# simonfuhrmann/mve

Hardware: NVIDIA H100
Metric: mvs_depth_pixels_per_second (higher is better)
Workload: dtype f32

## Files before the change

### mve_b200/csrc/patch_opt.cuh

```cuda
#pragma once
#if defined(B200MVS_HOST_EMU)
#include "simt_emu.h"
#else
#include <cuda_runtime.h>
#endif
#include <stdint.h>
#include <cstddef>

namespace b200mvs {

constexpr int MAX_LEVELS = 12;
constexpr int MAX_GLOBAL = 32;
constexpr int MAX_LOCAL = 4;
constexpr unsigned FULL = 0xffffffffu;
constexpr int NS = 25;
constexpr int CENTER = 12;
constexpr int LUT_REP = 32;
constexpr int LUT_STRIDE = 64;

struct alignas(16) LevelParams {
    float ax, ay, cx, cy;
    int w, h;
    int pitch;
    int pad;
    const uchar4* img;
    const uint4* quad;
};
static_assert(sizeof(LevelParams) == 48, "LevelParams layout");

struct alignas(16) ViewParams {
    float campos[3];
    float inv_ax0;
    float w2c[12];
    float rot[9];
    int nlevels;
    int valid;
    int pad;
    LevelParams lv[MAX_LEVELS];
};
static_assert(offsetof(ViewParams, lv) % 16 == 0, "ViewParams layout");

struct DevSettings {
    float min_ncc, min_parallax, accept_ncc, min_refine_diff;
    unsigned max_iterations, nr_recon_neighbors;
    int scale, use_color_scale;
};

struct JobParams {
    int ref_view, W, H, n_global;
    int gview[MAX_GLOBAL];
    float ki0, ki2, ki4, ki5;
    const uchar4* ref_img;
    int ref_pitch;
    int tiles_x;
    float* depth; float* conf; float* dz; float* normal;
    unsigned* slots;
    unsigned long long* sel;
    long long tile_base;
};

struct PatchIn  { int x, y; float depth, dzI, dzJ; unsigned slots; };
struct PatchOut { float conf, depth, dzI, dzJ, nx, ny, nz; unsigned slots; int iterations; int flags; };

#if defined(B200MVS_HOST_EMU)
__device__ __forceinline__ float rcp_fast(float x) { return 1.f / x; }
__device__ __forceinline__ float rsqrt_fast(float x) { return 1.f / sqrtf(x); }
#else
__device__ __forceinline__ float rcp_fast(float x) { float r; asm("rcp.approx.ftz.f32 %0, %1;" : "=f"(r) : "f"(x)); return r; }
__device__ __forceinline__ float rsqrt_fast(float x) { float r; asm("rsqrt.approx.ftz.f32 %0, %1;" : "=f"(r) : "f"(x)); return r; }
#endif

template <int K> __device__ __forceinline__ float lut_k(const float* table, unsigned lane4, unsigned w)
{
    static_assert(LUT_REP == 32 && LUT_STRIDE == 64, "offset arithmetic assumes 32 lanes and 256-byte rows");
#if defined(B200MVS_HOST_EMU)
    const unsigned off = (((w >> (8 * K)) & 0xFFu) << 8) | lane4;
#else
    const unsigned off = __byte_perm(w, lane4, 0x6504u | ((unsigned)K << 4));
#endif
    return *reinterpret_cast<const float*>(reinterpret_cast<const char*>(table) + off);
}

__device__ __forceinline__ float plx_weight(float p)
{
    if (p < 0.f || p > 180.f) return 0.f;
    const float sigma = (p <= 20.f) ? 5.f : 15.f;
    const float dlt = p - 20.f;
    return expf(-(dlt * dlt) / (2.f * sigma * sigma));
}
__device__ __forceinline__ float clamp1(float v) { return v < -1.f ? -1.f : (v > 1.f ? 1.f : v); }
__device__ __forceinline__ float deg_acos(float dp) { return acosf(dp) * 180.f / 3.141592653589793f; }

}
```

### mve_b200/csrc/patch_thread.cuh

```cuda
#pragma once
#include "patch_opt.cuh"

namespace b200mvs {

#if defined(B200MVS_SWEEP_MIX) && !defined(B200MVS_HOST_EMU)
__device__ unsigned long long g_sweep_mix[128];
__device__ __forceinline__ void count_sweep_mix(unsigned kind)
{
    const unsigned act = __activemask();
    const unsigned same = __match_any_sync(act, kind);
    const int lane = (int)(threadIdx.x & 31u);
    const unsigned firsts = __ballot_sync(act, (__ffs(same) - 1) == lane);
    atomicAdd(&g_sweep_mix[64 + (kind & 63u)], 1ull);
    if (lane == __ffs(act) - 1) {
        atomicAdd(&g_sweep_mix[__popc(firsts) & 31], 1ull);
        atomicAdd(&g_sweep_mix[32], 1ull);
        atomicAdd(&g_sweep_mix[33], (unsigned long long)__popc(act));
    }
}
#endif

struct PatchT {
    const DevSettings* st;
    const ViewParams* views;
#if defined(B200MVS_HOST_EMU)
    const float* lut_tab;
    unsigned lane4;
#endif
    const JobParams* job;
    unsigned xy;
    float u0x, u0y, u0z;
    float uax, uay, uaz;
    float ubx, uby, ubz;
    float c0x, c0y, c0z;
    float mx0, mx1, mx2;
    float crx, cry, crz;
    float cpx, cpy, cpz;
    float mfp, inv_mfp;
    float mm, inv_mm, sqrDevX;
    float depth, dzI, dzJ;
    unsigned avail;
    int iter;
    unsigned n_sets;
    unsigned pk;
    unsigned selp;
    float cs[MAX_LOCAL][3];
    float ncc[MAX_LOCAL];


    struct PassOut { float num, den, nX0, nX1, nX2; };
    enum Stage { LVS_CTOR, CTOR, FIRST, PRE, POST, LVS_REPL, REPL, DONE };
    enum : unsigned {
        F_REF_OK = 1u << 0,
        F_OPTI = 1u << 1, F_CONVERGED = 1u << 2, F_LVS_OK = 1u << 3, F_VIEW_REMOVED = 1u << 4, F_WAS_NORMAL = 1u << 5,
        F_NORMAL = 1u << 6, F_SINGULAR = 1u << 7, F_HAS_NORMAL = 1u << 8, F_HAS_NCC = 1u << 9
    };
    static constexpr int SH_STAGE = 10, SH_NSEL = 13, SH_COL = 16, SH_DER = 20, SH_DF = 24;
    __device__ __forceinline__ bool is(unsigned f) const { return (pk & f) != 0u; }
    __device__ __forceinline__ void put(unsigned f, bool v) { pk = v ? (pk | f) : (pk & ~f); }
    __device__ __forceinline__ int stage() const { return (int)((pk >> SH_STAGE) & 7u); }
    __device__ __forceinline__ void set_stage(int v) { pk = (pk & ~(7u << SH_STAGE)) | ((unsigned)v << SH_STAGE); }
    __device__ __forceinline__ int nsel() const { return (int)((pk >> SH_NSEL) & 7u); }
    __device__ __forceinline__ void set_nsel(int v) { pk = (pk & ~(7u << SH_NSEL)) | ((unsigned)v << SH_NSEL); }
    __device__ __forceinline__ int sel(int k) const { return (int)((selp >> (8 * k)) & 0xFFu); }
    __device__ __forceinline__ int px() const { return (int)(xy & 0xFFFFu); }
    __device__ __forceinline__ int py() const { return (int)(xy >> 16); }

    template <typename T> static __device__ __forceinline__ T get4(const T (&a)[MAX_LOCAL], int k)
    {
        return k == 0 ? a[0] : (k == 1 ? a[1] : (k == 2 ? a[2] : a[3]));
    }
    template <typename T> static __device__ __forceinline__ void set4(T (&a)[MAX_LOCAL], int k, T v)
    {
#pragma unroll
        for (int i = 0; i < MAX_LOCAL; ++i) if (i == k) a[i] = v;
    }

    __device__ __forceinline__ unsigned lane_offset() const
    {
#if defined(B200MVS_HOST_EMU)
        return lane4;
#else
        return (threadIdx.x & 31u) << 2;
#endif
    }
    __device__ __forceinline__ const float* table() const
    {
#if defined(B200MVS_HOST_EMU)
        return lut_tab;
#else
        extern __shared__ float b200mvs_dyn_smem[];
        return b200mvs_dyn_smem;
#endif
    }

    __device__ __forceinline__ void sample_ray(float di, float dj, float& ux, float& uy, float& uz, float& inv) const
    {
        ux = u0x + di * uax + dj * ubx;
        uy = u0y + di * uay + dj * uby;
        uz = u0z + di * uaz + dj * ubz;
        inv = rsqrt_fast(ux * ux + uy * uy + uz * uz);
    }

    __device__ __forceinline__ void compute_points()
    {
        bool bad = false;
#pragma unroll 5
        for (int k = 0; k < NS; ++k) {
            const float t = depth + (float)(k % 5 - 2) * dzI + (float)(k / 5 - 2) * dzJ;
            bad |= t <= 0.f;
        }
        if (bad) pk &= ~F_REF_OK;
        cpx = c0x + depth * crx;
        cpy = c0y + depth * cry;
        cpz = c0z + depth * crz;
        const ViewParams* rv = &views[job->ref_view];
        const float z = __ldg(&rv->w2c[8]) * cpx + __ldg(&rv->w2c[9]) * cpy + __ldg(&rv->w2c[10]) * cpz + __ldg(&rv->w2c[11]);
        mfp = z * job->ki0;
        inv_mfp = rcp_fast(mfp);
    }

    __device__ __forceinline__ void init_sampler(int x, int y)
    {
        const float* const lut_tab = table();
        const unsigned lane4 = lane_offset();
        pk &= ~F_REF_OK; mm = 0.f; inv_mm = 0.f; sqrDevX = 0.f;
        mx0 = mx1 = mx2 = 0.f;
        crx = cry = crz = cpx = cpy = cpz = mfp = inv_mfp = 0.f;
        if (x - 2 < 0 || y - 2 < 0 || x + 2 > job->W - 1 || y + 2 > job->H - 1) return;
        {
            const ViewParams* rv = &views[job->ref_view];
            const float r0 = __ldg(&rv->rot[0]), r1 = __ldg(&rv->rot[1]), r2 = __ldg(&rv->rot[2]), r3 = __ldg(&rv->rot[3]), r4 = __ldg(&rv->rot[4]);
            const float r5 = __ldg(&rv->rot[5]), r6 = __ldg(&rv->rot[6]), r7 = __ldg(&rv->rot[7]), r8 = __ldg(&rv->rot[8]);
            const float vx = job->ki0 * ((float)x + 0.5f) + job->ki2, vy = job->ki4 * ((float)y + 0.5f) + job->ki5;
            u0x = r0 * vx + r3 * vy + r6; u0y = r1 * vx + r4 * vy + r7; u0z = r2 * vx + r5 * vy + r8;
            uax = r0 * job->ki0; uay = r1 * job->ki0; uaz = r2 * job->ki0;
            ubx = r3 * job->ki4; uby = r4 * job->ki4; ubz = r5 * job->ki4;
            c0x = __ldg(&rv->campos[0]); c0y = __ldg(&rv->campos[1]); c0z = __ldg(&rv->campos[2]);
            const float inv = rsqrt_fast(u0x * u0x + u0y * u0y + u0z * u0z);
            crx = u0x * inv; cry = u0y * inv; crz = u0z * inv;
        }
        pk |= F_REF_OK;
        const uchar4* row = job->ref_img + (size_t)(y - 2) * job->ref_pitch + (x - 2);
        float s0 = 0.f, s1 = 0.f, s2 = 0.f;
#pragma unroll 1
        for (int j = 0; j < 5; ++j) {
#pragma unroll
            for (int i = 0; i < 5; ++i) {
                const unsigned t = reinterpret_cast<const unsigned*>(row)[i];
                s0 += lut_k<0>(lut_tab, lane4, t); s1 += lut_k<1>(lut_tab, lane4, t); s2 += lut_k<2>(lut_tab, lane4, t);
            }
            row += job->ref_pitch;
        }
        mm = (s0 + s1 + s2) / (3.f * NS);
        if (mm < 0.01f || mm > 0.99f) { pk &= ~F_REF_OK; return; }
        inv_mm = 1.f / mm;
        mx0 = (s0 * inv_mm) / (float)NS; mx1 = (s1 * inv_mm) / (float)NS; mx2 = (s2 * inv_mm) / (float)NS;
        row = job->ref_img + (size_t)(y - 2) * job->ref_pitch + (x - 2);
        float dev = 0.f;
#pragma unroll 1
        for (int j = 0; j < 5; ++j) {
#pragma unroll
            for (int i = 0; i < 5; ++i) {
                const unsigned t = reinterpret_cast<const unsigned*>(row)[i];
                const float e0 = lut_k<0>(lut_tab, lane4, t) * inv_mm - mx0, e1 = lut_k<1>(lut_tab, lane4, t) * inv_mm - mx1, e2 = lut_k<2>(lut_tab, lane4, t) * inv_mm - mx2;
                dev += e0 * e0 + e1 * e1 + e2 * e2;
            }
            row += job->ref_pitch;
        }
        sqrDevX = dev;
        compute_points();
    }

    __device__ __forceinline__ void update()
    {
        pk |= F_REF_OK;
        compute_points();
    }

    __device__ __forceinline__ void pass(bool candidates, bool cs_pending, bool want_ncc, bool want_normal, float* cand, PassOut& po)
    {
        const float* const lut_tab = table();
        const unsigned lane4 = lane_offset();
        const float u0x = this->u0x, u0y = this->u0y, u0z = this->u0z, uax = this->uax, uay = this->uay, uaz = this->uaz;
        const float ubx = this->ubx, uby = this->uby, ubz = this->ubz;
        const float depth = this->depth, dzI = this->dzI, dzJ = this->dzJ;
        const float inv_mm = this->inv_mm;
        const JobParams* const job = this->job;
        float num = 0.f, den = 0.f;
        double D0 = 0.0, D1 = 0.0, D2 = 0.0, D3 = 0.0, D4 = 0.0, D5 = 0.0, E0 = 0.0, E1 = 0.0, E2 = 0.0;
        bool cs_active = cs_pending && st->use_color_scale;
        if (!candidates) pk &= want_ncc ? ~((0xFFu << SH_COL) | (0xFu << SH_DF)) : ~(0xFFu << SH_COL);
        const int count = candidates ? job->n_global : nsel();
        const int x0 = px(), y0 = py();
        const float pv0 = mx0 * mm, pv1 = mx1 * mm, pv2 = mx2 * mm;
#pragma unroll 1
        for (int k = 0; k < count; ++k) {
            int slot = k;
            if (candidates) { if (!((avail >> k) & 1u)) continue; }
            else slot = sel(k);
            const ViewParams* V = &views[job->gview[slot]];
            ++n_sets;
            float c0 = 1.f, c1 = 1.f, c2 = 1.f;
            if (!candidates) {
                c0 = k == 0 ? cs[0][0] : (k == 1 ? cs[1][0] : (k == 2 ? cs[2][0] : cs[3][0]));
                c1 = k == 0 ? cs[0][1] : (k == 1 ? cs[1][1] : (k == 2 ? cs[2][1] : cs[3][1]));
                c2 = k == 0 ? cs[0][2] : (k == 1 ? cs[1][2] : (k == 2 ? cs[2][2] : cs[3][2]));
            }
            unsigned r = 0u;
            float A0x = 0.f, A0y = 0.f, A0z = 0.f, W0x = 0.f, W0y = 0.f, W0z = 0.f, Wax = 0.f, Way = 0.f, Waz = 0.f, Wbx = 0.f, Wby = 0.f, Wbz = 0.f;
            float Lax = 0.f, Lay = 0.f, Lcx = 0.f, Lcy = 0.f, wm1 = 0.f, hm1 = 0.f, dd = 0.f, step = 0.f;
            int Lpitch = 0;
            const uint4* Lquad = nullptr;
            bool dok = false;
            {
                const float4 wa = __ldg(reinterpret_cast<const float4*>(&V->w2c[0]));
                const float4 wb = __ldg(reinterpret_cast<const float4*>(&V->w2c[4]));
                const float4 wc = __ldg(reinterpret_cast<const float4*>(&V->w2c[8]));
                A0x = wa.x * c0x + wa.y * c0y + wa.z * c0z + wa.w;
                A0y = wb.x * c0x + wb.y * c0y + wb.z * c0z + wb.w;
                A0z = wc.x * c0x + wc.y * c0y + wc.z * c0z + wc.w;
                W0x = wa.x * u0x + wa.y * u0y + wa.z * u0z; W0y = wb.x * u0x + wb.y * u0y + wb.z * u0z; W0z = wc.x * u0x + wc.y * u0y + wc.z * u0z;
                Wax = wa.x * uax + wa.y * uay + wa.z * uaz; Way = wb.x * uax + wb.y * uay + wb.z * uaz; Waz = wc.x * uax + wc.y * uay + wc.z * uaz;
                Wbx = wa.x * ubx + wa.y * uby + wa.z * ubz; Wby = wb.x * ubx + wb.y * uby + wb.z * ubz; Wbz = wc.x * ubx + wc.y * uby + wc.z * ubz;
                const float nz = wc.x * cpx + wc.y * cpy + wc.z * cpz + wc.w;
                const float nfp = nz * __ldg(&V->inv_ax0);
                if (mfp > 0.f && !(nfp <= 0.f)) {
                    float ratio = nfp * inv_mfp;
                    int l = 0;
                    while (ratio < 0.5f) { ++l; ratio *= 2.f; }
                    const int nl = __ldg(&V->nlevels);
                    if (l > nl - 1) l = nl - 1;
                    const float4 kk = __ldg(reinterpret_cast<const float4*>(&V->lv[l].ax));
                    const int4 g = __ldg(reinterpret_cast<const int4*>(&V->lv[l].w));
                    Lax = kk.x; Lay = kk.y; Lcx = kk.z; Lcy = kk.w; wm1 = (float)(g.x - 1); hm1 = (float)(g.y - 1); Lpitch = g.z;
                    Lquad = reinterpret_cast<const uint4*>(__ldg(reinterpret_cast<const unsigned long long*>(&V->lv[l].quad)));
                    const float inv0 = rsqrt_fast(u0x * u0x + u0y * u0y + u0z * u0z);
                    const float sa = depth * inv0, sb = (depth + 1.f) * inv0;
                    const float hz1 = A0z + sa * W0z, hz2 = A0z + sb * W0z;
                    const float i1 = rcp_fast(hz1), i2 = rcp_fast(hz2);
                    const float ddx = (Lax * (A0x + sb * W0x) + Lcx * hz2) * i2 - (Lax * (A0x + sa * W0x) + Lcx * hz1) * i1;
                    const float ddy = (Lay * (A0y + sb * W0y) + Lcy * hz2) * i2 - (Lay * (A0y + sa * W0y) + Lcy * hz1) * i1;
                    const float dd2 = ddx * ddx + ddy * ddy;
                    dd = dd2 * rsqrt_fast(dd2);
                    dok = dd > 0.f;
                    step = rcp_fast(dd);
                    r = dok ? 3u : 1u;
                    if (!dok) dd = 0.f;
                }
            }
            const bool need_ncc = candidates || want_ncc;
            const bool cs_view = !candidates && cs_active;
            float nccv = -1.f;
#pragma unroll 1
            for (int rep = 0; rep < 2 && r != 0u; ++rep) {
                const bool second = rep == 1;
                if (second && !(cs_view && want_normal && (r & 2u))) break;
                const bool gn = !candidates && (r & 2u) && (second || !(cs_view && want_normal));
                const bool nrm = gn && want_normal;
#if defined(B200MVS_SWEEP_MIX) && !defined(B200MVS_HOST_EMU)
                {
                    const bool g_ = !candidates && (r & 2u);
                    count_sweep_mix((!second && need_ncc ? 1u : 0u) | (!second && cs_view ? 2u : 0u) |
                                    (g_ && !second && cs_view && !want_normal ? 4u : 0u) | (g_ && (second || !cs_view) ? 8u : 0u) |
                                    (g_ && (second || !cs_view) && want_normal ? 16u : 0u) | (candidates ? 32u : 0u));
                }
#endif
                float Sya = 0.f, Syb = 0.f, Syc = 0.f, Syya = 0.f, Syyb = 0.f, Syyc = 0.f, Smya = 0.f, Smyb = 0.f, Smyc = 0.f;
                float Sdma = 0.f, Sdmb = 0.f, Sdmc = 0.f, Sdna = 0.f, Sdnb = 0.f, Sdnc = 0.f, Sdda = 0.f, Sddb = 0.f, Sddc = 0.f;
                float A1 = 0.f, A2 = 0.f, A3 = 0.f, A4 = 0.f, A5 = 0.f, B1 = 0.f, B2 = 0.f;
                bool oob = false;
                const uchar4* mptr = job->ref_img + (size_t)(y0 - 2) * job->ref_pitch + (x0 - 2);
                const int mskip = job->ref_pitch - 5;
                float ndi = -2.f, ndj = -2.f;
                float nfx = 0.f, nfy = 0.f, ngx = 0.f, ngy = 0.f;
                uint4 nQ = make_uint4(0u, 0u, 0u, 0u);
                unsigned nmt = 0u;
                bool nvalid = false;
#define B200MVS_STAGE_NEXT() do { \
                    const float ux_ = u0x + ndi * uax + ndj * ubx, uy_ = u0y + ndi * uay + ndj * uby, uz_ = u0z + ndi * uaz + ndj * ubz; \
                    const float inv_ = rsqrt_fast(ux_ * ux_ + uy_ * uy_ + uz_ * uz_); \
                    const float t_ = depth + ndi * dzI + ndj * dzJ; \
                    const float s1_ = t_ * inv_; \
                    const float wx_ = W0x + ndi * Wax + ndj * Wbx, wy_ = W0y + ndi * Way + ndj * Wby, wz_ = W0z + ndi * Waz + ndj * Wbz; \
                    const float hx_ = A0x + s1_ * wx_, hy_ = A0y + s1_ * wy_, hz_ = A0z + s1_ * wz_; \
                    const float ih_ = rcp_fast(hz_); \
                    const float qx_ = (Lax * hx_ + Lcx * hz_) * ih_ - 0.5f; \
                    const float qy_ = (Lay * hy_ + Lcy * hz_) * ih_ - 0.5f; \
                    nvalid = qx_ > 0.f && qx_ < wm1 && qy_ > 0.f && qy_ < hm1; \
                    if (nvalid) { \
                        ngx = 0.f; ngy = 0.f; \
                        if (dok) { \
                            const float s2_ = s1_ + step * inv_; \
                            const float kx_ = A0x + s2_ * wx_, ky_ = A0y + s2_ * wy_, kz_ = A0z + s2_ * wz_; \
                            const float ik_ = rcp_fast(kz_); \
                            ngx = (Lax * kx_ + Lcx * kz_) * ik_ - 0.5f - qx_; \
                            ngy = (Lay * ky_ + Lcy * kz_) * ik_ - 0.5f - qy_; \
                        } \
                        const int left_ = (int)floorf(qx_), top_ = (int)floorf(qy_); \
                        nfx = qx_ - (float)left_; nfy = qy_ - (float)top_; \
                        noff = (unsigned)top_ * (unsigned)Lpitch + (unsigned)left_; \
                        nQ = __ldg(Lquad + noff); \
                        nmt = *reinterpret_cast<const unsigned*>(mptr); \
                    } \
                } while (0)
                unsigned noff = 0u;
                B200MVS_STAGE_NEXT();
#ifdef B200MVS_T1_UNROLL2
#pragma unroll 2
#else
#pragma unroll 1
#endif
                for (int k = 0; k < NS; ++k) {
                    if (!nvalid) { oob = true; break; }
                    const float di = ndi, dj = ndj, fx = nfx, fy = nfy, gx = ngx, gy = ngy;
                    const uint4 Q = nQ;
                    const unsigned mt = nmt;
                    if (k + 1 < NS) {
                        ndi += 1.f; ++mptr;
                        if (ndi > 2.f) { ndi = -2.f; ndj += 1.f; mptr += mskip; }
                        B200MVS_STAGE_NEXT();
                    }
                    {
                        const float m[3] = {lut_k<0>(lut_tab, lane4, mt) * inv_mm, lut_k<1>(lut_tab, lane4, mt) * inv_mm, lut_k<2>(lut_tab, lane4, mt) * inv_mm};
                        float a[3], b[3], c[3], e[3];
                        a[0] = lut_k<0>(lut_tab, lane4, Q.x); a[1] = lut_k<1>(lut_tab, lane4, Q.x); a[2] = lut_k<2>(lut_tab, lane4, Q.x);
                        b[0] = lut_k<0>(lut_tab, lane4, Q.y); b[1] = lut_k<1>(lut_tab, lane4, Q.y); b[2] = lut_k<2>(lut_tab, lane4, Q.y);
                        c[0] = lut_k<0>(lut_tab, lane4, Q.z); c[1] = lut_k<1>(lut_tab, lane4, Q.z); c[2] = lut_k<2>(lut_tab, lane4, Q.z);
                        e[0] = lut_k<0>(lut_tab, lane4, Q.w); e[1] = lut_k<1>(lut_tab, lane4, Q.w); e[2] = lut_k<2>(lut_tab, lane4, Q.w);
                        float n[3], d[3];
#pragma unroll
                        for (int ch = 0; ch < 3; ++ch) {
                            const float x0_ = (1.f - fx) * a[ch] + fx * b[ch];
                            const float x3_ = (1.f - fx) * c[ch] + fx * e[ch];
                            n[ch] = (1.f - fy) * x0_ + fy * x3_;
                            const float der = gx * (b[ch] - a[ch]) + gy * (c[ch] - a[ch]) + (gy * fx + gx * fy) * (a[ch] - b[ch] - c[ch] + e[ch]);
                            d[ch] = der * dd;
                        }
                        const float y0_ = n[0] - pv0, y1_ = n[1] - pv1, y2_ = n[2] - pv2;
                        Sya += y0_; Syb += y1_; Syc += y2_;
                        Syya += y0_ * y0_; Syyb += y1_ * y1_; Syyc += y2_ * y2_;
                        Smya += m[0] * y0_; Smyb += m[1] * y1_; Smyc += m[2] * y2_;
                        Sdma += d[0] * m[0]; Sdmb += d[1] * m[1]; Sdmc += d[2] * m[2];
                        Sdna += d[0] * n[0]; Sdnb += d[1] * n[1]; Sdnc += d[2] * n[2];
                        Sdda += d[0] * d[0]; Sddb += d[1] * d[1]; Sddc += d[2] * d[2];
                        if (nrm) {
                            const float g0 = c0 * d[0], g1 = c1 * d[1], g2 = c2 * d[2];
                            const float q = g0 * g0 + g1 * g1 + g2 * g2;
                            const float s = g0 * (m[0] - c0 * n[0]) + g1 * (m[1] - c1 * n[1]) + g2 * (m[2] - c2 * n[2]);
                            const float qi = di * q, qj = dj * q;
                            A1 += qi; A2 += qj; A3 += di * qi; A4 += dj * qi; A5 += dj * qj;
                            B1 += di * s; B2 += dj * s;
                        }
                    }
                }
#undef B200MVS_STAGE_NEXT
                if (oob) { r = 0u; break; }
                if (!second && need_ncc) {
                    const float inv_n = 1.f / (float)NS;
                    const float sqrDevY = (Syya - Sya * Sya * inv_n) + (Syyb - Syb * Syb * inv_n) + (Syyc - Syc * Syc * inv_n);
                    const float Sen = (Smya - mx0 * Sya) + (Smyb - mx1 * Syb) + (Smyc - mx2 * Syc);
                    const float p = sqrDevX * sqrDevY;
                    nccv = p > 0.f ? Sen * rsqrt_fast(p) : -1.f;
                }
                if (!second && cs_view) {
                    const float Mna = Smya + pv0 * ((float)NS * mx0), Mnb = Smyb + pv1 * ((float)NS * mx1), Mnc = Smyc + pv2 * ((float)NS * mx2);
                    const float Nna = Syya + pv0 * (2.f * Sya + (float)NS * pv0), Nnb = Syyb + pv1 * (2.f * Syb + (float)NS * pv1);
                    const float Nnc = Syyc + pv2 * (2.f * Syc + (float)NS * pv2);
                    float cc[3] = {c0, c1, c2};
                    const float ab[3] = {Mna - c0 * Nna, Mnb - c1 * Nnb, Mnc - c2 * Nnc};
                    const float aa[3] = {Nna, Nnb, Nnc};
#pragma unroll
                    for (int ch = 0; ch < 3; ++ch) {
                        if ((double)fabsf(aa[ch]) > 1e-6) {
                            cc[ch] += ab[ch] * rcp_fast(aa[ch]);
                            if ((double)cc[ch] > 1e3) pk &= ~F_OPTI;
                        } else
                            pk &= ~F_OPTI;
                    }
                    c0 = cc[0]; c1 = cc[1]; c2 = cc[2];
#pragma unroll
                    for (int i = 0; i < MAX_LOCAL; ++i) if (i == k) { cs[i][0] = c0; cs[i][1] = c1; cs[i][2] = c2; }
                }
                if (gn) {
                    const float vn = c0 * (Sdma - c0 * Sdna) + c1 * (Sdmb - c1 * Sdnb) + c2 * (Sdmc - c2 * Sdnc);
                    const float vd = c0 * c0 * Sdda + c1 * c1 * Sddb + c2 * c2 * Sddc;
                    num += vn; den += vd;
                    if (nrm) {
                        D0 += (double)vd; D1 += (double)A1; D2 += (double)A2; D3 += (double)A3; D4 += (double)A4; D5 += (double)A5;
                        E0 += (double)vn; E1 += (double)B1; E2 += (double)B2;
                    }
                }
            }
            if (!candidates) {
                if (r & 1u) pk |= 1u << (SH_COL + k);
                if (r & 2u) pk |= 1u << (SH_DER + k);
                if (cs_active && !(r & 1u)) cs_active = false;
                if (want_ncc) {
                    const float v = (r & 1u) ? nccv : -1.f;
                    if (fabsf(v - get4(ncc, k)) > st->min_refine_diff) pk |= 1u << (SH_DF + k);
                    set4(ncc, k, v);
                }
            } else {
                const float v = (r & 1u) ? nccv : -1.f;
                if (v < st->min_ncc) avail &= ~(1u << k);
                else cand[k] = v;
            }
        }
        if (candidates) return;
        po.num = num; po.den = den;
        put(F_HAS_NORMAL, want_normal);
        put(F_HAS_NCC, want_ncc);
        if (want_normal) {
            const double m[9] = {D0, D1, D2, D1, D3, D4, D2, D4, D5};
            const double det = m[0] * m[4] * m[8] + m[1] * m[5] * m[6] + m[2] * m[3] * m[7]
                             - m[2] * m[4] * m[6] - m[1] * m[3] * m[8] - m[0] * m[5] * m[7];
            put(F_SINGULAR, det == 0.0);
            double inv[9];
            inv[0] = m[4] * m[8] - m[5] * m[7];
            inv[1] = m[2] * m[7] - m[1] * m[8];
            inv[2] = m[1] * m[5] - m[2] * m[4];
            inv[3] = m[5] * m[6] - m[3] * m[8];
            inv[4] = m[0] * m[8] - m[2] * m[6];
            inv[5] = m[2] * m[3] - m[0] * m[5];
            inv[6] = m[3] * m[7] - m[4] * m[6];
            inv[7] = m[1] * m[6] - m[0] * m[7];
            inv[8] = m[0] * m[4] - m[1] * m[3];
#pragma unroll
            for (int q = 0; q < 9; ++q) inv[q] /= det;
            po.nX0 = (float)(inv[0] * E0 + inv[1] * E1 + inv[2] * E2);
            po.nX1 = (float)(inv[3] * E0 + inv[4] * E1 + inv[5] * E2);
            po.nX2 = (float)(inv[6] * E0 + inv[7] * E1 + inv[8] * E2);
        }
    }

    __device__ __forceinline__ bool all_der_ok() const { return ((pk >> SH_DER) & 0xFu) == ((1u << nsel()) - 1u); }

    __device__ __forceinline__ bool depth_step(const PassOut& po)
    {
        if (!all_der_ok()) { pk &= ~F_OPTI; return false; }
        if (po.den > 0.f) {
            depth += po.num / po.den;
            update();
            put(F_OPTI, is(F_REF_OK));
            return true;
        }
        return false;
    }

    __device__ __forceinline__ bool normal_step(const PassOut& po)
    {
        if (!all_der_ok()) { pk &= ~F_OPTI; return false; }
        if (is(F_SINGULAR)) { pk &= ~F_OPTI; return false; }
        dzI += po.nX1; dzJ += po.nX2; depth += po.nX0;
        update();
        put(F_OPTI, is(F_REF_OK));
        return true;
    }

    __device__ __forceinline__ void sel_erase_mask(unsigned mask)
    {
        const int n = nsel();
        int cnt = 0;
        unsigned packed = 0xFFFFFFFFu;
#pragma unroll
        for (int k = 0; k < MAX_LOCAL; ++k) {
            if (k < n && !((mask >> k) & 1u)) {
                const unsigned s8 = (selp >> (8 * k)) & 0xFFu;
                const float a = cs[k][0], b = cs[k][1], c = cs[k][2], v = ncc[k];
                packed = (packed & ~(0xFFu << (8 * cnt))) | (s8 << (8 * cnt));
#pragma unroll
                for (int q = 0; q < MAX_LOCAL; ++q) if (q == cnt) { cs[q][0] = a; cs[q][1] = b; cs[q][2] = c; ncc[q] = v; }
                ++cnt;
            }
        }
        selp = packed;
        set_nsel(cnt);
    }
    __device__ __forceinline__ void sel_insert(int slot, float cs_init)
    {
        const int n = nsel();
        int pos = 0;
#pragma unroll
        for (int k = 0; k < MAX_LOCAL; ++k) if (k < n && sel(k) < slot) ++pos;
#pragma unroll
        for (int q = MAX_LOCAL - 1; q > 0; --q)
            if (q > pos && q <= n) { cs[q][0] = cs[q - 1][0]; cs[q][1] = cs[q - 1][1]; cs[q][2] = cs[q - 1][2]; ncc[q] = ncc[q - 1]; }
#pragma unroll
        for (int q = 0; q < MAX_LOCAL; ++q) if (q == pos) { cs[q][0] = cs[q][1] = cs[q][2] = cs_init; ncc[q] = 0.f; }
        const unsigned low = pos == 0 ? 0u : (selp & (0xFFFFFFFFu >> (32 - 8 * pos)));
        const unsigned high = pos >= 3 ? 0u : ((selp >> (8 * pos)) << (8 * (pos + 1)));
        selp = low | ((unsigned)slot << (8 * pos)) | high;
        set_nsel(n + 1);
    }

    __device__ __forceinline__ void cand_geometry(int slot, float rdx, float rdy, float rdz,
                                                  float& vdx, float& vdy, float& vdz, float& epx, float& epy, float& epz, float& nfp) const
    {
        const ViewParams* V = &views[job->gview[slot]];
        vdx = cpx - __ldg(&V->campos[0]); vdy = cpy - __ldg(&V->campos[1]); vdz = cpz - __ldg(&V->campos[2]);
        const float nn = sqrtf(vdx * vdx + vdy * vdy + vdz * vdz);
        vdx /= nn; vdy /= nn; vdz /= nn;
        epx = vdy * rdz - vdz * rdy; epy = vdz * rdx - vdx * rdz; epz = vdx * rdy - vdy * rdx;
        const float en = sqrtf(epx * epx + epy * epy + epz * epz);
        epx /= en; epy /= en; epz /= en;
        const float z = __ldg(&V->w2c[8]) * cpx + __ldg(&V->w2c[9]) * cpy + __ldg(&V->w2c[10]) * cpz + __ldg(&V->w2c[11]);
        nfp = z * __ldg(&V->inv_ax0);
    }

    __device__ __forceinline__ void lvs_greedy(const float* cand)
    {
        const unsigned N = st->nr_recon_neighbors;
        const float cs_init = 1.f / mm;
        float rdx = cpx - c0x, rdy = cpy - c0y, rdz = cpz - c0z;
        {
            const float nn = sqrtf(rdx * rdx + rdy * rdy + rdz * rdz);
            rdx /= nn; rdy /= nn; rdz /= nn;
        }
        const int G = job->n_global;
        bool found = true;
        while ((unsigned)nsel() < N && found) {
            found = false;
            float maxScore = 0.f;
            int maxView = 0;
#pragma unroll 1
            for (int c = 0; c < G; ++c) {
                if (!((avail >> c) & 1u)) continue;
                float vdx, vdy, vdz, epx, epy, epz, nfp;
                cand_geometry(c, rdx, rdy, rdz, vdx, vdy, vdz, epx, epy, epz, nfp);
                float score = cand[c];
                if (mfp / nfp < 0.5f) score *= 0.01f;
                float dp = clamp1(rdx * vdx + rdy * vdy + rdz * vdz);
                score *= plx_weight(deg_acos(dp));
                const int ns = nsel();
#pragma unroll 1
                for (int k = 0; k < ns; ++k) {
                    float sx, sy, sz, ex, ey, ez, sfp;
                    cand_geometry(sel(k), rdx, rdy, rdz, sx, sy, sz, ex, ey, ez, sfp);
                    dp = clamp1(sx * vdx + sy * vdy + sz * vdz);
                    score *= plx_weight(deg_acos(dp));
                    dp = clamp1(epx * ex + epy * ey + epz * ez);
                    float angle = fabsf(deg_acos(dp));
                    if (angle > 90.f) angle = 180.f - angle;
                    angle = fmaxf(angle, 1.f);
                    if (angle < st->min_parallax) score *= angle / st->min_parallax;
                }
                if (score > maxScore) { maxScore = score; maxView = c; found = true; }
            }
            if (found) {
                sel_insert(maxView, cs_init);
                avail &= ~(1u << maxView);
            }
        }
        if ((unsigned)nsel() == N) pk |= F_LVS_OK;
    }

    __device__ __forceinline__ void begin(const JobParams* j, const PatchIn& in)
    {
        job = j;
        xy = ((unsigned)in.x & 0xFFFFu) | ((unsigned)in.y << 16);
        depth = in.depth; dzI = in.dzI; dzJ = in.dzJ;
        iter = 0;
        pk = F_OPTI | F_SINGULAR | ((unsigned)DONE << SH_STAGE);
        avail = 0u;
        u0x = u0y = u0z = uax = uay = uaz = ubx = uby = ubz = c0x = c0y = c0z = 0.f;
        init_sampler(in.x, in.y);
        selp = in.slots;
        int n = 0;
#pragma unroll
        for (int k = 0; k < MAX_LOCAL; ++k) {
            if (sel(k) != 0xFF) n = k + 1;
            cs[k][0] = cs[k][1] = cs[k][2] = 0.f; ncc[k] = 0.f;
        }
        set_nsel(n);
        if (!is(F_REF_OK)) { pk &= ~F_OPTI; return; }
        const unsigned N = st->nr_recon_neighbors;
        if ((unsigned)n == N) pk |= F_LVS_OK;
        else if ((unsigned)n > N) {
            n = 0;
            set_nsel(0);
            selp = 0xFFFFFFFFu;
        }
        avail = job->n_global >= 32 ? FULL : ((1u << job->n_global) - 1u);
#pragma unroll
        for (int k = 0; k < MAX_LOCAL; ++k) if (k < n) avail &= ~(1u << sel(k));
        const float ci = 1.f / mm;
#pragma unroll
        for (int k = 0; k < MAX_LOCAL; ++k) { cs[k][0] = cs[k][1] = cs[k][2] = ci; }
        set_stage(is(F_LVS_OK) ? CTOR : LVS_CTOR);
    }

    __device__ __forceinline__ bool step()
    {
        int stage = this->stage();
        if (stage == DONE) return true;
        const bool a_cand = (stage == LVS_CTOR) | (stage == LVS_REPL);
        const bool a_cs = (stage == CTOR) | (stage == REPL) | ((stage == POST) & is(F_WAS_NORMAL));
        const bool a_ncc = (stage == PRE) | (stage == POST) | (stage == REPL) | ((stage == FIRST) & (iter == 4));
        const bool a_normal = (stage == REPL) | ((stage == FIRST) & (iter == 4)) | ((stage == PRE) & is(F_NORMAL)) |
                              ((stage == POST) & ((iter + 1) % 5 == 4));
        float cand[MAX_GLOBAL];
        PassOut po = {0.f, 0.f, 0.f, 0.f, 0.f};
        pass(a_cand, a_cs, a_ncc, a_normal, cand, po);
        if (stage == LVS_CTOR || stage == LVS_REPL) {
            lvs_greedy(cand);
            if (!is(F_LVS_OK)) { if (stage == LVS_CTOR) pk &= ~F_OPTI; set_stage(DONE); return true; }
            set_stage((stage == LVS_CTOR) ? CTOR : REPL);
            return false;
        }
        if (!is(F_OPTI)) { set_stage(DONE); return true; }
        if (stage == POST) {
            const int n = nsel();
            const unsigned dfb = (pk >> SH_DF) & ((1u << n) - 1u);
            unsigned tbr = (iter == 14) ? dfb : 0u;
#pragma unroll
            for (int k = 0; k < MAX_LOCAL; ++k)
                if (k < n && ncc[k] < st->accept_ncc) tbr |= 1u << k;
            if (tbr) {
                pk |= F_VIEW_REMOVED;
                sel_erase_mask(tbr);
                pk &= ~F_LVS_OK;
                set_stage(LVS_REPL);
                return false;
            }
            if (dfb == 0u) { pk |= F_CONVERGED; set_stage(DONE); return true; }
            ++iter;
        } else if (stage == REPL) {
            ++iter;
        }
        while (iter < 4 && is(F_OPTI)) {
            const bool moved = depth_step(po);
            ++iter;
            if (moved && is(F_OPTI)) { set_stage(FIRST); return false; }
        }
        if (!is(F_OPTI)) { set_stage(DONE); return true; }
        if (!((unsigned)iter < st->max_iterations && is(F_LVS_OK))) { set_stage(DONE); return true; }
        const bool normal = (iter % 5 == 4) || is(F_VIEW_REMOVED);
        put(F_NORMAL, normal);
        if (!is(F_HAS_NCC) || (normal && !is(F_HAS_NORMAL))) { set_stage(PRE); return false; }
        pk &= ~F_OPTI;
        if (normal) { normal_step(po); pk &= ~F_VIEW_REMOVED; pk |= F_WAS_NORMAL; }
        else { depth_step(po); pk &= ~F_WAS_NORMAL; }
        if (!is(F_OPTI)) { set_stage(DONE); return true; }
        set_stage(POST);
        return false;
    }

    __device__ __forceinline__ void finish(PatchOut& out)
    {
        out.depth = depth; out.dzI = dzI; out.dzJ = dzJ;
        out.iterations = iter;
        out.flags = (is(F_CONVERGED) ? 1 : 0) | (is(F_OPTI) ? 2 : 0);
        const int n = nsel();
        out.slots = n >= 4 ? selp : (selp | (0xFFFFFFFFu << (8 * n)));
        out.conf = 0.f; out.nx = out.ny = out.nz = 0.f;
        if (!is(F_CONVERGED)) return;
        float mean = 0.f;
#pragma unroll
        for (int k = 0; k < MAX_LOCAL; ++k) if (k < n) mean += ncc[k];
        mean /= (float)n;
        const float score = (mean - st->accept_ncc) / (1.f - st->accept_ncc);
        float px[4], py[4], pz[4];
        const float di_[4] = {2.f, -2.f, 0.f, 0.f}, dj_[4] = {0.f, 0.f, -2.f, 2.f};
#pragma unroll
        for (int q = 0; q < 4; ++q) {
            float ux, uy, uz, inv;
            sample_ray(di_[q], dj_[q], ux, uy, uz, inv);
            const float s1 = (depth + di_[q] * dzI + dj_[q] * dzJ) * inv;
            px[q] = c0x + s1 * ux; py[q] = c0y + s1 * uy; pz[q] = c0z + s1 * uz;
        }
        const float ax_ = px[0] - px[1], ay_ = py[0] - py[1], az_ = pz[0] - pz[1];
        const float bx_ = px[2] - px[3], by_ = py[2] - py[3], bz_ = pz[2] - pz[3];
        float nx = ay_ * bz_ - az_ * by_, ny = az_ * bx_ - ax_ * bz_, nz = ax_ * by_ - ay_ * bx_;
        const float nn = sqrtf(nx * nx + ny * ny + nz * nz);
        nx /= nn; ny /= nn; nz /= nn;
        out.nx = nx; out.ny = ny; out.nz = nz;
        const float dotP = -(nx * crx + ny * cry + nz * crz);
        out.conf = (dotP < 0.2f) ? 0.f : score;
    }
};

#if !defined(B200MVS_HOST_EMU)
static_assert(sizeof(PatchT) % 16 == 8 && sizeof(PatchT) <= 248, "PatchT stride in shared memory must be 8 mod 16 bytes, and 512 of them must fit beside the table");
#endif

__device__ __forceinline__ void bind_thread(PatchT& p, const DevSettings* st, const ViewParams* views, const float* lut_rep, int tid)
{
    p.st = st; p.views = views;
#if defined(B200MVS_HOST_EMU)
    p.lut_tab = lut_rep; p.lane4 = 4u * (unsigned)(tid & (LUT_REP - 1));
#else
    (void)lut_rep; (void)tid;
#endif
    p.pk = (unsigned)PatchT::DONE << PatchT::SH_STAGE;
    p.n_sets = 0u;
}

}
```

Baseline: 61.39 million.

## Restructure patch sweep into two-deep staged pipeline with branchless out-of-bounds handling

Replaces the macro-based one-ahead prefetch loop over the 25 patch samples with a Sweep struct that keeps two staged samples in flight, processing two per iteration. Out-of-bounds samples no longer break early; coordinates are clamped to zero and validity is AND-accumulated, then checked after the sweep. Arithmetic is rewritten with explicit round-to-nearest fma/mul/add intrinsics. The aim is more memory-level parallelism on the quad texture loads and fewer divergent branches, at the cost of higher register pressure, extra work on invalid views and slightly different floating-point rounding.

Measured after the change: 67.28 million, median of 6. 1.1x the previous value.

```diff
diff --git a/mve_b200/csrc/patch_opt.cuh b/mve_b200/csrc/patch_opt.cuh
--- a/mve_b200/csrc/patch_opt.cuh
+++ b/mve_b200/csrc/patch_opt.cuh
@@ -65,9 +65,17 @@
 #if defined(B200MVS_HOST_EMU)
 __device__ __forceinline__ float rcp_fast(float x) { return 1.f / x; }
 __device__ __forceinline__ float rsqrt_fast(float x) { return 1.f / sqrtf(x); }
+__device__ __forceinline__ float fma_rn(float a, float b, float c) { return a * b + c; }
+__device__ __forceinline__ float mul_rn(float a, float b) { return a * b; }
+__device__ __forceinline__ float add_rn(float a, float b) { return a + b; }
+__device__ __forceinline__ float sub_rn(float a, float b) { return a - b; }
 #else
 __device__ __forceinline__ float rcp_fast(float x) { float r; asm("rcp.approx.ftz.f32 %0, %1;" : "=f"(r) : "f"(x)); return r; }
 __device__ __forceinline__ float rsqrt_fast(float x) { float r; asm("rsqrt.approx.ftz.f32 %0, %1;" : "=f"(r) : "f"(x)); return r; }
+__device__ __forceinline__ float fma_rn(float a, float b, float c) { return __fmaf_rn(a, b, c); }
+__device__ __forceinline__ float mul_rn(float a, float b) { return __fmul_rn(a, b); }
+__device__ __forceinline__ float add_rn(float a, float b) { return __fadd_rn(a, b); }
+__device__ __forceinline__ float sub_rn(float a, float b) { return __fsub_rn(a, b); }
 #endif
 
 template <int K> __device__ __forceinline__ float lut_k(const float* table, unsigned lane4, unsigned w)
diff --git a/mve_b200/csrc/patch_thread.cuh b/mve_b200/csrc/patch_thread.cuh
--- a/mve_b200/csrc/patch_thread.cuh
+++ b/mve_b200/csrc/patch_thread.cuh
@@ -1,5 +1,8 @@
 #pragma once
 #include "patch_opt.cuh"
+#if defined(B200MVS_HOST_EMU)
+#include <cassert>
+#endif
 
 namespace b200mvs {
 
@@ -177,6 +180,105 @@
         pk |= F_REF_OK;
         compute_points();
     }
+
+    struct Staged {
+        uint4 Q;
+        unsigned mt;
+        float fx, fy, gx, gy;
+    };
+    struct Sweep {
+        const float* lut;
+        unsigned lane4;
+        float inv_mm;
+        float u0x, u0y, u0z, uax, uay, uaz, ubx, uby, ubz, depth, dzI, dzJ;
+        float A0x, A0y, A0z, W0x, W0y, W0z, Wax, Way, Waz, Wbx, Wby, Wbz;
+        float Lax, Lay, Lcx, Lcy, wm1, hm1, step, dd;
+        const uint4* quad;
+        unsigned qpitch;
+        const uchar4* master;
+        int mpitch;
+        float pv0, pv1, pv2;
+        float c0, c1, c2;
+        bool nrm;
+        float Sya, Syb, Syc, Syya, Syyb, Syyc, Smya, Smyb, Smyc;
+        float Sdma, Sdmb, Sdmc, Sdna, Sdnb, Sdnc, Sdda, Sddb, Sddc;
+        float A1, A2, A3, A4, A5, B1, B2;
+
+        __device__ __forceinline__ void clear()
+        {
+            Sya = Syb = Syc = Syya = Syyb = Syyc = Smya = Smyb = Smyc = 0.f;
+            Sdma = Sdmb = Sdmc = Sdna = Sdnb = Sdnc = Sdda = Sddb = Sddc = 0.f;
+            A1 = A2 = A3 = A4 = A5 = B1 = B2 = 0.f;
+        }
+
+        __device__ __forceinline__ bool stage(int k, Staged& s) const
+        {
+            const int row = k / 5, col = k - 5 * row;
+            const float di = (float)(col - 2), dj = (float)(row - 2);
+            const float ux = fma_rn(dj, ubx, fma_rn(di, uax, u0x)), uy = fma_rn(dj, uby, fma_rn(di, uay, u0y)), uz = fma_rn(dj, ubz, fma_rn(di, uaz, u0z));
+            const float inv = rsqrt_fast(fma_rn(uz, uz, fma_rn(ux, ux, mul_rn(uy, uy))));
+            const float s1 = mul_rn(fma_rn(dj, dzJ, fma_rn(di, dzI, depth)), inv);
+            const float wx = fma_rn(dj, Wbx, fma_rn(di, Wax, W0x)), wy = fma_rn(dj, Wby, fma_rn(di, Way, W0y)), wz = fma_rn(dj, Wbz, fma_rn(di, Waz, W0z));
+            const float hx = fma_rn(s1, wx, A0x), hy = fma_rn(s1, wy, A0y), hz = fma_rn(s1, wz, A0z);
+            const float ih = rcp_fast(hz);
+            const float qx = fma_rn(fma_rn(Lax, hx, mul_rn(Lcx, hz)), ih, -0.5f);
+            const float qy = fma_rn(fma_rn(Lay, hy, mul_rn(Lcy, hz)), ih, -0.5f);
+            const bool ok = qx > 0.f && qx < wm1 && qy > 0.f && qy < hm1;
+            const float s2 = fma_rn(step, inv, s1);
+            const float kx = fma_rn(s2, wx, A0x), ky = fma_rn(s2, wy, A0y), kz = fma_rn(s2, wz, A0z);
+            const float ik = rcp_fast(kz);
+            s.gx = sub_rn(fma_rn(fma_rn(Lax, kx, mul_rn(Lcx, kz)), ik, -0.5f), qx);
+            s.gy = sub_rn(fma_rn(fma_rn(Lay, ky, mul_rn(Lcy, kz)), ik, -0.5f), qy);
+            const float cx = ok ? qx : 0.f, cy = ok ? qy : 0.f;
+            const int left = (int)floorf(cx), top = (int)floorf(cy);
+#if defined(B200MVS_HOST_EMU)
+            assert(left >= 0 && top >= 0 && (float)left < wm1 && (float)top < hm1);
+#endif
+            s.fx = sub_rn(cx, (float)left);
+            s.fy = sub_rn(cy, (float)top);
+            s.Q = __ldg(quad + ((unsigned)top * qpitch + (unsigned)left));
+            s.mt = *reinterpret_cast<const unsigned*>(master + row * mpitch + col);
+            return ok;
+        }
+
+        __device__ __forceinline__ void sample(int k, const Staged& in)
+        {
+            const float fx = in.fx, fy = in.fy, gx = in.gx, gy = in.gy;
+            const float m[3] = {mul_rn(lut_k<0>(lut, lane4, in.mt), inv_mm), mul_rn(lut_k<1>(lut, lane4, in.mt), inv_mm), mul_rn(lut_k<2>(lut, lane4, in.mt), inv_mm)};
+            float a[3], b[3], c[3], e[3];
+            a[0] = lut_k<0>(lut, lane4, in.Q.x); a[1] = lut_k<1>(lut, lane4, in.Q.x); a[2] = lut_k<2>(lut, lane4, in.Q.x);
+            b[0] = lut_k<0>(lut, lane4, in.Q.y); b[1] = lut_k<1>(lut, lane4, in.Q.y); b[2] = lut_k<2>(lut, lane4, in.Q.y);
+            c[0] = lut_k<0>(lut, lane4, in.Q.z); c[1] = lut_k<1>(lut, lane4, in.Q.z); c[2] = lut_k<2>(lut, lane4, in.Q.z);
+            e[0] = lut_k<0>(lut, lane4, in.Q.w); e[1] = lut_k<1>(lut, lane4, in.Q.w); e[2] = lut_k<2>(lut, lane4, in.Q.w);
+            const float omfx = sub_rn(1.f, fx), omfy = sub_rn(1.f, fy), wxy = fma_rn(fy, gx, mul_rn(fx, gy));
+            float n[3], d[3];
+#pragma unroll
+            for (int ch = 0; ch < 3; ++ch) {
+                const float x0 = fma_rn(omfx, a[ch], mul_rn(fx, b[ch]));
+                const float x3 = fma_rn(omfx, c[ch], mul_rn(fx, e[ch]));
+                n[ch] = fma_rn(omfy, x0, mul_rn(fy, x3));
+                const float t = fma_rn(gx, sub_rn(b[ch], a[ch]), mul_rn(gy, sub_rn(c[ch], a[ch])));
+                d[ch] = mul_rn(fma_rn(wxy, add_rn(sub_rn(sub_rn(a[ch], b[ch]), c[ch]), e[ch]), t), dd);
+            }
+            const float y0 = sub_rn(n[0], pv0), y1 = sub_rn(n[1], pv1), y2 = sub_rn(n[2], pv2);
+            Sya = add_rn(Sya, y0); Syb = add_rn(Syb, y1); Syc = add_rn(Syc, y2);
+            Syya = fma_rn(y0, y0, Syya); Syyb = fma_rn(y1, y1, Syyb); Syyc = fma_rn(y2, y2, Syyc);
+            Smya = fma_rn(m[0], y0, Smya); Smyb = fma_rn(m[1], y1, Smyb); Smyc = fma_rn(m[2], y2, Smyc);
+            Sdma = fma_rn(d[0], m[0], Sdma); Sdmb = fma_rn(d[1], m[1], Sdmb); Sdmc = fma_rn(d[2], m[2], Sdmc);
+            Sdna = fma_rn(d[0], n[0], Sdna); Sdnb = fma_rn(d[1], n[1], Sdnb); Sdnc = fma_rn(d[2], n[2], Sdnc);
+            Sdda = fma_rn(d[0], d[0], Sdda); Sddb = fma_rn(d[1], d[1], Sddb); Sddc = fma_rn(d[2], d[2], Sddc);
+            if (nrm) {
+                const int row = k / 5;
+                const float di = (float)(k - 5 * row - 2), dj = (float)(row - 2);
+                const float g0 = mul_rn(c0, d[0]), g1 = mul_rn(c1, d[1]), g2 = mul_rn(c2, d[2]);
+                const float q = fma_rn(g2, g2, fma_rn(g0, g0, mul_rn(g1, g1)));
+                const float s = fma_rn(g2, fma_rn(-c2, n[2], m[2]), fma_rn(g0, fma_rn(-c0, n[0], m[0]), mul_rn(g1, fma_rn(-c1, n[1], m[1]))));
+                const float qi = mul_rn(di, q), qj = mul_rn(dj, q);
+                A1 = add_rn(A1, qi); A2 = add_rn(A2, qj); A3 = fma_rn(di, qi, A3); A4 = fma_rn(dj, qi, A4); A5 = fma_rn(dj, qj, A5);
+                B1 = fma_rn(di, s, B1); B2 = fma_rn(dj, s, B2);
+            }
+        }
+    };
 
     __device__ __forceinline__ void pass(bool candidates, bool cs_pending, bool want_ncc, bool want_normal, float* cand, PassOut& po)
     {
@@ -212,7 +314,6 @@
             float Lax = 0.f, Lay = 0.f, Lcx = 0.f, Lcy = 0.f, wm1 = 0.f, hm1 = 0.f, dd = 0.f, step = 0.f;
             int Lpitch = 0;
             const uint4* Lquad = nullptr;
-            bool dok = false;
             {
                 const float4 wa = __ldg(reinterpret_cast<const float4*>(&V->w2c[0]));
                 const float4 wb = __ldg(reinterpret_cast<const float4*>(&V->w2c[4]));
@@ -243,10 +344,8 @@
                     const float ddy = (Lay * (A0y + sb * W0y) + Lcy * hz2) * i2 - (Lay * (A0y + sa * W0y) + Lcy * hz1) * i1;
                     const float dd2 = ddx * ddx + ddy * ddy;
                     dd = dd2 * rsqrt_fast(dd2);
-                    dok = dd > 0.f;
                     step = rcp_fast(dd);
-                    r = dok ? 3u : 1u;
-                    if (!dok) dd = 0.f;
+                    r = dd > 0.f ? 3u : 1u;
                 }
             }
             const bool need_ncc = candidates || want_ncc;
@@ -266,96 +365,36 @@
                                     (g_ && (second || !cs_view) && want_normal ? 16u : 0u) | (candidates ? 32u : 0u));
                 }
 #endif
-                float Sya = 0.f, Syb = 0.f, Syc = 0.f, Syya = 0.f, Syyb = 0.f, Syyc = 0.f, Smya = 0.f, Smyb = 0.f, Smyc = 0.f;
-                float Sdma = 0.f, Sdmb = 0.f, Sdmc = 0.f, Sdna = 0.f, Sdnb = 0.f, Sdnc = 0.f, Sdda = 0.f, Sddb = 0.f, Sddc = 0.f;
-                float A1 = 0.f, A2 = 0.f, A3 = 0.f, A4 = 0.f, A5 = 0.f, B1 = 0.f, B2 = 0.f;
-                bool oob = false;
-                const uchar4* mptr = job->ref_img + (size_t)(y0 - 2) * job->ref_pitch + (x0 - 2);
-                const int mskip = job->ref_pitch - 5;
-                float ndi = -2.f, ndj = -2.f;
-                float nfx = 0.f, nfy = 0.f, ngx = 0.f, ngy = 0.f;
-                uint4 nQ = make_uint4(0u, 0u, 0u, 0u);
-                unsigned nmt = 0u;
-                bool nvalid = false;
-#define B200MVS_STAGE_NEXT() do { \
-                    const float ux_ = u0x + ndi * uax + ndj * ubx, uy_ = u0y + ndi * uay + ndj * uby, uz_ = u0z + ndi * uaz + ndj * ubz; \
-                    const float inv_ = rsqrt_fast(ux_ * ux_ + uy_ * uy_ + uz_ * uz_); \
-                    const float t_ = depth + ndi * dzI + ndj * dzJ; \
-                    const float s1_ = t_ * inv_; \
-                    const float wx_ = W0x + ndi * Wax + ndj * Wbx, wy_ = W0y + ndi * Way + ndj * Wby, wz_ = W0z + ndi * Waz + ndj * Wbz; \
-                    const float hx_ = A0x + s1_ * wx_, hy_ = A0y + s1_ * wy_, hz_ = A0z + s1_ * wz_; \
-                    const float ih_ = rcp_fast(hz_); \
-                    const float qx_ = (Lax * hx_ + Lcx * hz_) * ih_ - 0.5f; \
-                    const float qy_ = (Lay * hy_ + Lcy * hz_) * ih_ - 0.5f; \
-                    nvalid = qx_ > 0.f && qx_ < wm1 && qy_ > 0.f && qy_ < hm1; \
-                    if (nvalid) { \
-                        ngx = 0.f; ngy = 0.f; \
-                        if (dok) { \
-                            const float s2_ = s1_ + step * inv_; \
-                            const float kx_ = A0x + s2_ * wx_, ky_ = A0y + s2_ * wy_, kz_ = A0z + s2_ * wz_; \
-                            const float ik_ = rcp_fast(kz_); \
-                            ngx = (Lax * kx_ + Lcx * kz_) * ik_ - 0.5f - qx_; \
-                            ngy = (Lay * ky_ + Lcy * kz_) * ik_ - 0.5f - qy_; \
-                        } \
-                        const int left_ = (int)floorf(qx_), top_ = (int)floorf(qy_); \
-                        nfx = qx_ - (float)left_; nfy = qy_ - (float)top_; \
-                        noff = (unsigned)top_ * (unsigned)Lpitch + (unsigned)left_; \
-                        nQ = __ldg(Lquad + noff); \
-                        nmt = *reinterpret_cast<const unsigned*>(mptr); \
-                    } \
-                } while (0)
-                unsigned noff = 0u;
-                B200MVS_STAGE_NEXT();
-#ifdef B200MVS_T1_UNROLL2
-#pragma unroll 2
-#else
+                Sweep sw;
+                sw.lut = lut_tab; sw.lane4 = lane4; sw.inv_mm = inv_mm;
+                sw.u0x = u0x; sw.u0y = u0y; sw.u0z = u0z; sw.uax = uax; sw.uay = uay; sw.uaz = uaz; sw.ubx = ubx; sw.uby = uby; sw.ubz = ubz;
+                sw.depth = depth; sw.dzI = dzI; sw.dzJ = dzJ;
+                sw.A0x = A0x; sw.A0y = A0y; sw.A0z = A0z; sw.W0x = W0x; sw.W0y = W0y; sw.W0z = W0z;
+                sw.Wax = Wax; sw.Way = Way; sw.Waz = Waz; sw.Wbx = Wbx; sw.Wby = Wby; sw.Wbz = Wbz;
+                sw.Lax = Lax; sw.Lay = Lay; sw.Lcx = Lcx; sw.Lcy = Lcy; sw.wm1 = wm1; sw.hm1 = hm1; sw.step = step; sw.dd = dd;
+                sw.quad = Lquad; sw.qpitch = (unsigned)Lpitch;
+                sw.master = job->ref_img + (size_t)(y0 - 2) * job->ref_pitch + (x0 - 2); sw.mpitch = job->ref_pitch;
+                sw.pv0 = pv0; sw.pv1 = pv1; sw.pv2 = pv2; sw.c0 = c0; sw.c1 = c1; sw.c2 = c2; sw.nrm = nrm;
+                sw.clear();
+                Staged sa, sb;
+                bool ok = sw.stage(0, sa);
+                ok &= sw.stage(1, sb);
 #pragma unroll 1
-#endif
-                for (int k = 0; k < NS; ++k) {
-                    if (!nvalid) { oob = true; break; }
-                    const float di = ndi, dj = ndj, fx = nfx, fy = nfy, gx = ngx, gy = ngy;
-                    const uint4 Q = nQ;
-                    const unsigned mt = nmt;
-                    if (k + 1 < NS) {
-                        ndi += 1.f; ++mptr;
-                        if (ndi > 2.f) { ndi = -2.f; ndj += 1.f; mptr += mskip; }
-                        B200MVS_STAGE_NEXT();
-                    }
-                    {
-                        const float m[3] = {lut_k<0>(lut_tab, lane4, mt) * inv_mm, lut_k<1>(lut_tab, lane4, mt) * inv_mm, lut_k<2>(lut_tab, lane4, mt) * inv_mm};
-                        float a[3], b[3], c[3], e[3];
-                        a[0] = lut_k<0>(lut_tab, lane4, Q.x); a[1] = lut_k<1>(lut_tab, lane4, Q.x); a[2] = lut_k<2>(lut_tab, lane4, Q.x);
-                        b[0] = lut_k<0>(lut_tab, lane4, Q.y); b[1] = lut_k<1>(lut_tab, lane4, Q.y); b[2] = lut_k<2>(lut_tab, lane4, Q.y);
-                        c[0] = lut_k<0>(lut_tab, lane4, Q.z); c[1] = lut_k<1>(lut_tab, lane4, Q.z); c[2] = lut_k<2>(lut_tab, lane4, Q.z);
-                        e[0] = lut_k<0>(lut_tab, lane4, Q.w); e[1] = lut_k<1>(lut_tab, lane4, Q.w); e[2] = lut_k<2>(lut_tab, lane4, Q.w);
-                        float n[3], d[3];
-#pragma unroll
-                        for (int ch = 0; ch < 3; ++ch) {
-                            const float x0_ = (1.f - fx) * a[ch] + fx * b[ch];
-                            const float x3_ = (1.f - fx) * c[ch] + fx * e[ch];
-                            n[ch] = (1.f - fy) * x0_ + fy * x3_;
-                            const float der = gx * (b[ch] - a[ch]) + gy * (c[ch] - a[ch]) + (gy * fx + gx * fy) * (a[ch] - b[ch] - c[ch] + e[ch]);
-                            d[ch] = der * dd;
-                        }
-                        const float y0_ = n[0] - pv0, y1_ = n[1] - pv1, y2_ = n[2] - pv2;
-                        Sya += y0_; Syb += y1_; Syc += y2_;
-                        Syya += y0_ * y0_; Syyb += y1_ * y1_; Syyc += y2_ * y2_;
-                        Smya += m[0] * y0_; Smyb += m[1] * y1_; Smyc += m[2] * y2_;
-                        Sdma += d[0] * m[0]; Sdmb += d[1] * m[1]; Sdmc += d[2] * m[2];
-                        Sdna += d[0] * n[0]; Sdnb += d[1] * n[1]; Sdnc += d[2] * n[2];
-                        Sdda += d[0] * d[0]; Sddb += d[1] * d[1]; Sddc += d[2] * d[2];
-                        if (nrm) {
-                            const float g0 = c0 * d[0], g1 = c1 * d[1], g2 = c2 * d[2];
-                            const float q = g0 * g0 + g1 * g1 + g2 * g2;
-                            const float s = g0 * (m[0] - c0 * n[0]) + g1 * (m[1] - c1 * n[1]) + g2 * (m[2] - c2 * n[2]);
-                            const float qi = di * q, qj = dj * q;
-                            A1 += qi; A2 += qj; A3 += di * qi; A4 += dj * qi; A5 += dj * qj;
-                            B1 += di * s; B2 += dj * s;
-                        }
-                    }
+                for (int k = 0; k < NS - 3; k += 2) {
+                    sw.sample(k, sa);
+                    ok &= sw.stage(k + 2, sa);
+                    sw.sample(k + 1, sb);
+                    ok &= sw.stage(k + 3, sb);
                 }
-#undef B200MVS_STAGE_NEXT
-                if (oob) { r = 0u; break; }
+                sw.sample(NS - 3, sa);
+                ok &= sw.stage(NS - 1, sa);
+                sw.sample(NS - 2, sb);
+                sw.sample(NS - 1, sa);
+                const float Sya = sw.Sya, Syb = sw.Syb, Syc = sw.Syc, Syya = sw.Syya, Syyb = sw.Syyb, Syyc = sw.Syyc;
+                const float Smya = sw.Smya, Smyb = sw.Smyb, Smyc = sw.Smyc, Sdma = sw.Sdma, Sdmb = sw.Sdmb, Sdmc = sw.Sdmc;
+                const float Sdna = sw.Sdna, Sdnb = sw.Sdnb, Sdnc = sw.Sdnc, Sdda = sw.Sdda, Sddb = sw.Sddb, Sddc = sw.Sddc;
+                const float A1 = sw.A1, A2 = sw.A2, A3 = sw.A3, A4 = sw.A4, A5 = sw.A5, B1 = sw.B1, B2 = sw.B2;
+                if (!ok) { r = 0u; break; }
                 if (!second && need_ncc) {
                     const float inv_n = 1.f / (float)NS;
                     const float sqrDevY = (Syya - Sya * Sya * inv_n) + (Syyb - Syb * Syb * inv_n) + (Syyc - Syc * Syc * inv_n);
```
